# pigimonaco/Pinocchio

Measured on AMD Instinct MI355X. Metric: grid-cells/sec for full Fmax sweep (all smoothing radii) + 3LPT, 1024^3 box, higher is better.
Workload: dtype f64

## Files before the change

include/pinfmax.h:

```cpp
#ifndef PINFMAX_H
#define PINFMAX_H

#include <stddef.h>
#include <stdint.h>

#ifdef __cplusplus
extern "C" {
#endif

#define PF_NBINS 210
#define PF_MAX_SMOOTH 64

typedef struct pf_ctx pf_ctx;

typedef struct {
  int64_t n;
  int     rank;
  int     nranks;
  int     device;
  int     field_bytes;
  int     flags;
} pf_config;

#define PF_FLAG_TIMING 1
// ... 212 lines not shown
int pf_debug_pk(int which, const float *a, const float *b, float *out, int count);
int pf_debug_gfft(int n, int dir, const double *in, double *out);
int pf_debug_gfft_lines(int n, int mode, int dir, int nlines, const double *in, double *out);
int pf_debug_strided_jobs(int field_bytes, int n, int njobs, int nin, const int *in_of, const int *mul, int nouter, int ncols,
                          const double *in, double *out);
int pf_debug_strided_band(int field_bytes, int n, int njobs, int nin, const int *in_of, const int *mul, int nouter, int ncols,
                          int in_pitch, int out_pitch, int band_e, int band_outer, int outer_offset, int pre, double rs, double growth,
                          const double *in, double *out, int *guard_ok);
int pf_debug_zpass_jobs(int field_bytes, int n, int form, int njobs, const int *mul, const int *out_f32, int in_place, int nrows, int band,
                        double norm, const double *dc, int ncu, const double *spec, const double *hess, const double *acc, double *out,
                        int *sentinel_ok);
int pf_debug_strided_xfuse(int field_bytes, int n, int njobs, const int *mul, int nouter, int ncols, int pre, double rs, double growth,
                           int outer_offset, const double *in, double *out_fused, double *out_plain);
int pf_debug_invariant_reruns(pf_ctx *ctx);
int pf_solve_ran_beside_zpass(pf_ctx *ctx);
int pf_transform_path(pf_ctx *ctx);
int pf_invgrow_table_status(pf_ctx *ctx, int ismooth, double *max_rel_err);
int pf_collapse_cells(pf_ctx *ctx, int ismooth, const double *d, size_t count, double *F);
enum { PF_ARITH_FAST = 0, PF_ARITH_EXACT = 1 };
int pf_set_arithmetic(pf_ctx *ctx, int flavour);
int pf_get_arithmetic(pf_ctx *ctx);
#define PF_CENSUS_BINS 64
typedef struct {
  unsigned long long cells;
  unsigned long long differing_bits;
  unsigned long long hist[PF_CENSUS_BINS];
  unsigned long long beyond_2ulp;
  unsigned long long rmax_differing;
  unsigned long long nonfinite;
  unsigned long long outliers;
// ... 95 lines not shown
```

pinocchio_amd/_lib.py:

```python
from __future__ import annotations

import ctypes as C
import os

PKG = os.path.dirname(os.path.abspath(__file__))
SO = os.environ.get("PINFMAX_LIB") or os.path.join(PKG, "libpinfmax_hip.so")
NBINS = 210
MAX_SMOOTH = 64

FLAG_TIMING = 1
FLAG_DOUBLE_PRODUCTS = 2
MAP_CURRENT = 0
MAP_UPDATE = 1
NEIGH_SKIP, NEIGH_GOOD, NEIGH_PEAK = 1, 2, 4


class Config(C.Structure):
    _fields_ = [("n", C.c_int64), ("rank", C.c_int), ("nranks", C.c_int), ("device", C.c_int),
                ("field_bytes", C.c_int), ("flags", C.c_int)]


class ProductLayout(C.Structure):
    _fields_ = [("stride", C.c_size_t), ("off_Rmax", C.c_int), ("off_Fmax", C.c_int), ("off_Vel", C.c_int),
                ("off_Vel_2LPT", C.c_int), ("off_Vel_3LPT_1", C.c_int), ("off_Vel_3LPT_2", C.c_int)]
# ... 246 lines not shown
    "pf_debug_math": (C.c_int, [_vp, C.c_int, C.POINTER(C.c_double), C.POINTER(C.c_double), C.c_size_t, C.POINTER(C.c_double)]),
    "pf_debug_stream_rate": (C.c_int, [_vp, C.c_int, C.c_int, _dp]),
    "pf_debug_lines": (C.c_int, [C.c_int, C.c_int, C.c_int, C.c_int, C.c_int, C.c_int, C.c_int, C.c_int, C.c_double, C.c_double, C.c_int, _dp, _dp]),
    "pf_debug_pk": (C.c_int, [C.c_int, C.POINTER(C.c_float), C.POINTER(C.c_float), C.POINTER(C.c_float), C.c_int]),
    "pf_debug_gfft": (C.c_int, [C.c_int, C.c_int, _dp, _dp]),
    "pf_debug_gfft_lines": (C.c_int, [C.c_int, C.c_int, C.c_int, C.c_int, _dp, _dp]),
    "pf_debug_strided_jobs": (C.c_int, [C.c_int, C.c_int, C.c_int, C.c_int, C.POINTER(C.c_int), C.POINTER(C.c_int), C.c_int, C.c_int, _dp, _dp]),
    "pf_debug_strided_band": (C.c_int, [C.c_int, C.c_int, C.c_int, C.c_int, C.POINTER(C.c_int), C.POINTER(C.c_int), C.c_int, C.c_int, C.c_int, C.c_int,
                                        C.c_int, C.c_int, C.c_int, C.c_int, C.c_double, C.c_double, _dp, _dp, C.POINTER(C.c_int)]),
    "pf_debug_zpass_jobs": (C.c_int, [C.c_int, C.c_int, C.c_int, C.c_int, C.POINTER(C.c_int), C.POINTER(C.c_int), C.c_int, C.c_int, C.c_int, C.c_double,
                                      _dp, C.c_int, _dp, _dp, _dp, _dp, C.POINTER(C.c_int)]),
    "pf_debug_strided_xfuse": (C.c_int, [C.c_int, C.c_int, C.c_int, C.POINTER(C.c_int), C.c_int, C.c_int, C.c_int, C.c_double, C.c_double, C.c_int,
                                         _dp, _dp, _dp]),
    "pf_debug_invariant_reruns": (C.c_int, [_vp]),
    "pf_solve_ran_beside_zpass": (C.c_int, [_vp]),
    "pf_transform_path": (C.c_int, [_vp]),
    "pf_invgrow_table_status": (C.c_int, [_vp, C.c_int, _dp]),
    "pf_set_loopback_exchange": (C.c_int, [_vp, C.c_int]),
    "pf_loopback_active": (C.c_int, [_vp]),
    "pf_set_sources_in_sweep": (C.c_int, [_vp, C.c_int]),
    "pf_set_lpt_order": (C.c_int, [_vp, C.c_int]),
    "pf_set_ct_interpolation": (C.c_int, [_vp, C.c_int]),
    "pf_set_transposed_spectra": (C.c_int, [_vp, C.c_int]),
    "pf_replicated_spectrum": (C.c_int, [_vp]),
    "pf_update_products": (C.c_int, [_vp, _vp, C.POINTER(ProductLayout)]),
    "pf_set_growth_table": (C.c_int, [_vp, C.c_int, C.POINTER(C.c_double), C.c_int, C.c_double, C.c_double, C.c_double]),
    "pf_get_second_derivative": (C.c_int, [_vp, C.c_int, _dp]),
    "pf_get_kvector": (C.c_int, [_vp, C.c_int, _dp]),
    "pf_get_density": (C.c_int, [_vp, _dp]),
    "pf_debug_replicated_rows": (C.c_int, [_vp, C.c_int, C.c_int, _dp]),
# ... 73 lines not shown
```

pinocchio_amd/csrc/pf_api.hip:

```cpp
#include <hip/hip_runtime.h>

#include <math.h>
#include <stdarg.h>
#include <stdio.h>
#include <stdlib.h>
#include <string.h>

#include <atomic>
#include <string>
#include <functional>
#include <vector>

#include "../../include/pinfmax.h"
#include "pf_collapse_core.h"
#include "pf_hostpool.h"
#include "pf_internal.h"

extern "C" void pf_rccl_release(void *link);
extern "C" int pf_rccl_link_count(void *link);

static thread_local char g_err[512] = "";
int pf_fail(int task, const char *fmt, ...) {
  va_list ap;
  va_start(ap, fmt);
// ... 110 lines not shown
  int tab_ns;
  double tab_var[PF_MAX_SMOOTH];
  bool tab_ready;
  int tab_ismooth;
  int tab_built_fast;
  int model;
  double sng_cosmo[7], sng_Din[PF_MAX_SMOOTH], sng_size[PF_MAX_SMOOTH];
  int sng_ns;
  PfCtDev ct;
  double *ct_block;
  bool have_density, have_hessian, have_sources, products_init;
  int sources_order;
  bool sweep_sources, sources_fresh;
  bool x_pending[3];
  bool s3b_start_absent;
  bool transposed;
  int ct_flavour;
  int lpt_order;
  void *plc = nullptr;
  double *partials_src;
  bool general;
  void *W;
  void *fft_c2r, *fft_r2c;
  bool vel_zero_pending;
  int last_ns;
  struct PfHandoff *handoff;
  PfLoopback *loopback;
  pf_alltoall_fn a2a; void *a2a_user;
  pf_alltoallv_fn a2av; void *a2av_user;
  pf_allreduce_fn ared; void *ared_user;
// ... 110 lines not shown
  t->spline_lut = env_int("PF_SPLINE_LUT", 1) != 0;
  t->exchange_rows = env_int("PF_EXCHANGE_ROWS", 1) != 0;
  t->invariants = env_int("PF_INVARIANTS", 1);
  t->lpt_fuse = env_int("PF_LPT_FUSE", 1);
  t->collapse_wg_per_cu = env_int("PF_COLLAPSE_WG_PER_CU", 8);
  if (t->collapse_wg_per_cu <= 0) t->collapse_wg_per_cu = 8;
  t->general = env_int("PF_GENERAL", 0) != 0;

  t->pipeline = env_int("PF_PIPELINE", 1) != 0;
  t->replicate = env_int("PF_REPLICATE_DK", -1);
  t->exact_libm = env_int("PF_EXACT_LIBM", 0) != 0;
  t->solve_beside_z = env_int("PF_SOLVE_BESIDE_Z", -1);
  t->gtab = env_int("PF_GTAB", 1) != 0;
  t->lpt_xfuse = env_int("PF_LPT_XFUSE", 1) != 0;
  t->lpt3b_start = env_int("PF_LPT3B_START", 0) != 0;
  t->preflight = env_int("PF_PREFLIGHT", 1) != 0;
  t->handoff_chunk_mb = env_int("PF_HANDOFF_CHUNK_MB", 256);
  if (t->handoff_chunk_mb <= 0) t->handoff_chunk_mb = 256;
  t->handoff_threads = env_int("PF_HANDOFF_THREADS", 0);
  t->host_register = env_int("PF_HOST_REGISTER", 0) != 0;
  t->distribute_lds = env_int("PF_DISTRIBUTE_LDS", 1) != 0;
  const char *fault = getenv("PF_DEBUG_PIPELINE_FAULT");
  t->debug_fault = !fault ? 0 : !strcmp(fault, "recv") ? 1 : !strcmp(fault, "send") ? 2 : 0;
  t->prune_eps = 8.673617379884035e-19;
  if (const char *e = getenv("PF_PRUNE_EPS")) t->prune_eps = atof(e);
}

static void plan_bytes(const pf_ctx *c, size_t *at_create, size_t *peak) {
  const size_t field = c->field_bytes, nc = ncell_of(c);
  size_t fields = 1 + 3 + 6 + 3;
// ... 132 lines not shown
    return pf_fail(rank, "pf_create: PF_FLAG_DOUBLE_PRODUCTS (fp64 Fmax and displacements) needs fp64 fields");
  int ndev = 0;
  if (hipGetDeviceCount(&ndev) != hipSuccess || ndev <= 0)
    return pf_fail(rank, "pf_create: no HIP device available (libpinfmax_hip has no CPU path)");
  if (cfg->device < 0 || cfg->device >= ndev) return pf_fail(rank, "pf_create: device %d out of range (%d devices)", cfg->device, ndev);
  pf_ctx *c = new pf_ctx();
  c->cfg = *cfg; c->rank = rank; c->P = cfg->nranks; c->n = (int)n; c->nzh = c->n / 2 + 1; c->nzp = c->n / 2 + 64 / cfg->field_bytes;
  c->tune = tune; c->dev = cfg->device; c->inv_reruns = 0;
  c->general = want_general; c->fft_c2r = c->fft_r2c = nullptr; c->W = nullptr;
  if (c->general) c->nzp = c->nzh;
  c->nxl = c->n / c->P; c->nyl = c->n / c->P; c->fb = cfg->field_bytes; c->timing = (cfg->flags & PF_FLAG_TIMING) != 0; c->pb = (cfg->flags & PF_FLAG_DOUBLE_PRODUCTS) ? 8 : 4;
  c->dev_bytes = 0; c->own_stream = true; c->stream = nullptr;
  c->a2a = nullptr; c->a2av = nullptr; c->a2av_user = nullptr; c->ared = nullptr; c->a2a_user = c->ared_user = nullptr; c->rccl = nullptr;
  c->have_density = c->have_hessian = c->have_sources = c->products_init = false; c->last_ns = 0;
  c->sweep_sources = c->sources_fresh = false; c->x_pending[0] = c->x_pending[1] = c->x_pending[2] = false; c->s3b_start_absent = false; c->partials_src = nullptr; c->lpt_order = 3; c->ct_flavour = 0; c->transposed = false;
  c->vel_zero_pending = false; c->have_genic = false;
  memset(c->ks_ms, 0, sizeof(c->ks_ms)); memset(c->ks_bytes, 0, sizeof(c->ks_bytes)); memset(c->ks_n, 0, sizeof(c->ks_n));
  memset(&c->cpu, 0, sizeof(c->cpu)); memset(c->spl_set, 0, sizeof(c->spl_set)); memset(c->spl_n, 0, sizeof(c->spl_n));
  c->growth[0] = 1.0; c->growth[1] = 3. / 7.; c->growth[2] = -1. / 9.; c->growth[3] = 5. / 42.;
  for (int i = 0; i < 6; i++) { c->B[i] = nullptr; c->B2[i] = nullptr; }
  c->blockA = nullptr; c->dk = nullptr; c->recvA = nullptr; c->tw = nullptr;
  c->blockA2 = nullptr; c->recvA2 = nullptr; c->cstream = nullptr; c->dk_full = nullptr; c->replicate = false; c->dk_full_valid = false; for (int k = 0; k < 3; k++) c->INV[0][k] = c->INV[1][k] = nullptr; c->inv_w = 0; c->inv_own[0] = c->inv_own[1] = nullptr; c->blockS = c->blockB2 = nullptr;
  c->fmax = nullptr; c->rmax = nullptr; c->vel12 = nullptr; c->back_zacc = nullptr; c->back_group = nullptr; c->vel12_prev = nullptr; c->prev_shifts = 0; c->have_displacements = false; c->partials = nullptr; c->scal = nullptr; c->hist = nullptr; c->spl = nullptr;
  c->gtab = nullptr; c->etab = nullptr; c->ct_block = nullptr; c->gt = nullptr; c->gt_lut = nullptr;
  memset(c->gt_ok, 0, sizeof(c->gt_ok)); memset(c->gt_err, 0, sizeof(c->gt_err));
  for (int i = 0; i < 2; i++) c->ev_x[i] = c->ev_r[i] = c->ev_y[i] = c->ev_s[i] = nullptr;
  c->sstream = nullptr; c->solve_ran_beside = false; c->loopback = nullptr; c->handoff = nullptr;
  c->pipeline = c->P > 1 && tune.pipeline;
  for (int i = 0; i < 3; i++) { c->A[i] = nullptr; c->S[i] = nullptr; }
  memset(c->gt_n, 0, sizeof(c->gt_n));
  c->tab_ns = 0; c->tab_ready = false; c->tab_ismooth = -1; c->tab_built_fast = -1; c->model = 0; c->sng_ns = 0; memset(c->sng_cosmo, 0, sizeof(c->sng_cosmo)); memset(c->sng_size, 0, sizeof(c->sng_size)); memset(&c->ct, 0, sizeof(c->ct));
// ... 327 lines not shown
    }
    KTimer t(c, KS_ZPASS_INV, njobs * frac_in * spec_bytes_alg(c) + 3.0 * (double)ncell(c) * 8.0);
    PFCHK(c, pf_launch_c2r_invariants(c->fb, c->n, p, c->stream));
    return 0;
  }
  KTimer t(c, kind, njobs * frac_in * spec_bytes_alg(c) + outb);
  PFCHK(c, pf_launch_c2r(c->fb, c->n, p, c->stream));
  return 0;
}

__global__ void k_debug_idle(long long ticks) {
  const long long t0 = wall_clock64();
  while (wall_clock64() - t0 < ticks) __builtin_amdgcn_s_sleep(32);
}
template <class Pre, class Dst, class Post, class Band>
static int pipelined_band(pf_ctx *c, int count, int nf, Pre pre, Dst dst, Post post, Band band, bool local = false) {
  void *A[2][3];
  const void *R[3];
  if (local) {
    for (int i = 0; i < count; i++) {
      void *D[3];
      for (int f = 0; f < nf; f++) { D[f] = dst(i, 0, f); R[f] = D[f]; }
      if (pre(i, D)) return 1;
      if (post(i, R)) return 1;
    }
    return 0;
  }
  for (int f = 0; f < 3; f++) { A[0][f] = c->A[f]; A[1][f] = c->pipeline ? (void *)(c->blockA2 + f * c->field_bytes) : c->A[f]; }
  if (c->P == 1 || !c->pipeline) {
    for (int i = 0; i < count; i++) {
      if (pre(i, A[0])) return 1;
      for (int f = 0; f < nf; f++) {
        R[f] = A[0][f];
        if (c->P > 1) { void *d = dst(i, 0, f); PFCHK(c, exchange_band(c, A[0][f], d, band(i))); R[f] = d; }
      }
      if (post(i, R)) return 1;
    }
    return 0;
  }
  auto issue = [&](int i) -> int {
    const int s = i & 1;
    if (c->tune.debug_fault == 2) hipLaunchKernelGGL(k_debug_idle, dim3(1), dim3(1), 0, c->stream, 200000LL);
    if (pre(i, A[s])) return 1;
    HIPCHK(c, hipEventRecord(c->ev_x[s], c->stream));
    if (c->tune.debug_fault != 2) HIPCHK(c, hipStreamWaitEvent(c->cstream, c->ev_x[s], 0));
// ... 80 lines not shown
    const double kb = kc * c->n / (2.0 * 3.14159265358979323846);
    if (kb < c->n / 2 - 1) band = (int)kb + 1;
  }
  return band;
}
static int x_pending_of(const pf_ctx *c, const void *spec) {
  for (int i = 0; i < 3; i++) if (c->x_pending[i] && spec == c->S[i]) return i;
  return -1;
}
static int finish_forward_x(pf_ctx *c, int i) {
  const Job xj[1] = {{c->S[i], c->S[i], PF_MUL_ONE}};
  PFCHK(c, xpass(c, KS_XPASS_FWD, -1, 1, xj, 0, 0.0, 1.0, 1));
  c->x_pending[i] = false;
  return 0;
}
static int hess_x(pf_ctx *c, const void *spec, double rs, void *const A[3], int band, bool replicated = false) {
  const Job xj[3] = {{spec, A[0], PF_MUL_ONE}, {spec, A[1], PF_MUL_K}, {spec, A[2], PF_MUL_K2}};
  int pend = replicated ? -1 : x_pending_of(c, spec);
  if (pend >= 0 && band < c->n / 2) { PFCHK(c, finish_forward_x(c, pend)); pend = -1; }
  return xpass(c, KS_XPASS_HESS, +1, 3, xj, 1, rs, 1.0, 1, band, true, replicated, pend >= 0);
}
static int ensure_dk_full(pf_ctx *c) {
  if (!c->replicate || c->dk_full_valid) return 0;
  if (c->a2a == loopback_a2a && c->have_genic) {
    unsigned int *dseed = nullptr;
    const int rc = pf_genic_launch(c->fb, c->dk_full, c->n, c->nzp, c->n, 0, &c->genic, c->stream, &dseed);
    if (!rc) HIPCHK(c, hipStreamSynchronize(c->stream));
    hipFree(dseed);
    if (rc) return pf_fail(c->rank, "pf_genic_density (whole spectrum): launch failed");
    c->dk_full_valid = true;
    return 0;
  }
  const size_t rows = (size_t)c->nyl * c->nzp * 2 * c->fb;
  HIPCHK(c, hipMemsetAsync(c->dk_full, 0, (size_t)c->P * c->field_bytes, c->stream));
  HIPCHK(c, hipMemcpy2DAsync((char *)c->dk_full + (size_t)c->rank * rows, (size_t)c->P * rows, c->dk, rows, rows, (size_t)c->n,
                             hipMemcpyDeviceToDevice, c->stream));
  PFCHK(c, allreduce_dev(c, c->dk_full, (size_t)c->P * c->field_bytes / 8, 1));
  c->dk_full_valid = true;
  return 0;
}
static int hess_yz(pf_ctx *c, const void *const R[3], const double *dc, void *const out[6], int band, bool invariants = false,
                   void *acc = nullptr, void *const *hfirst = nullptr, bool in_local = false, const std::function<int()> *between = nullptr) {
  const Job yj[6] = {{R[2], out[0], PF_MUL_ONE}, {R[1], out[3], PF_MUL_K}, {R[1], out[4], PF_MUL_ONE},
                     {R[0], out[1], PF_MUL_K2}, {R[0], out[5], PF_MUL_K},  {R[0], out[2], PF_MUL_ONE}};
  PFCHK(c, ypass(c, KS_YPASS_HESS, +1, 6, yj, true, false, 3, band, true, in_local));
  if (between && (*between)()) return 1;
  const ZJob zj[6] = {{out[0], out[0], PF_MUL_ONE, 0}, {out[1], out[1], PF_MUL_ONE, 0}, {out[2], out[2], PF_MUL_K2, 0},
                      {out[3], out[3], PF_MUL_ONE, 0}, {out[4], out[4], PF_MUL_K, 0},   {out[5], out[5], PF_MUL_K, 0}};
  if (acc) {
    ZJob cj[6];
    for (int i = 0; i < 6; i++) { cj[i] = zj[i]; cj[i].out = hfirst[i]; }
    PFCHK(c, zpass_c2r(c, KS_ZPASS_HESS, 6, cj, dc, band, false, acc));
    return 0;
  }
  PFCHK(c, zpass_c2r(c, KS_ZPASS_HESS, 6, zj, dc, band, invariants));
  return 0;
}
static int hessian_of(pf_ctx *c, const void *spec, double rs, const double *dc, void *const out[6],
                      void *acc = nullptr, void *const *hfirst = nullptr) {
  if (c->general) return g_hessian_of(c, spec, rs, out);
// ... 149 lines not shown
static int dc_of_host_spec(pf_ctx *c, const double *host, int slot) {
  const double dcv = (c->rank == 0) ? host[0] / ((double)c->n * c->n * c->n) : 0.0;
  HIPCHK(c, hipMemcpyAsync(c->scal + slot, &dcv, sizeof(double), hipMemcpyHostToDevice, c->stream));
  HIPCHK(c, hipStreamSynchronize(c->stream));
  PFCHK(c, allreduce_dev(c, c->scal + slot, 1, 0));
  HIPCHK(c, hipStreamSynchronize(c->stream));
  return 0;
}

extern "C" int pf_set_density(pf_ctx *c, const double *kd) {
  if (!c || !kd) return pf_fail(0, "pf_set_density: null argument");
  PhaseTimer pt(c, 3);
  PFCHK(c, import_spec(c, kd, c->dk));
  PFCHK(c, dc_of_host_spec(c, kd, SC_DC_DK));
  c->have_genic = false;
  c->have_density = true; c->have_hessian = false; c->have_sources = false; c->sources_fresh = false; c->dk_full_valid = false;
  return 0;
}

extern "C" int pf_synth_density(pf_ctx *c, uint64_t seed, double sigma0, double slope) {
  if (!c) return 1;
  if (c->general) {
    PFCHK(c, pf_launch_white(c->fb, c->B[0], (long long)c->n * c->n, 0, c->n, c->n, seed, c->stream));
    PFCHK(c, g_r2c(c, c->B[0], c->dk));
  } else {
    PFCHK(c, pf_launch_white(c->fb, c->dk, (long long)c->nxl * c->n, (long long)c->rank * c->nxl * c->n, c->n, 2 * c->nzp, seed, c->stream));
    PFCHK(c, forward_of(c, c->dk));
  }
  PfShapeParams p; memset(&p, 0, sizeof(p));
  p.spec = c->dk; p.n = c->n; p.nzp = c->nzp; p.nyl = c->nyl; p.y0 = c->rank * c->nyl; p.slope = slope; p.scale = 1.0;
  p.partials = c->partials; p.nblocks = PF_NBLK; p.mode = 0; p.dscale = nullptr;
  PFCHK(c, pf_launch_shape(c->fb, p, c->stream));
  PFCHK(c, pf_launch_sum1(c->partials, PF_NBLK, 1.0, c->scal + SC_POWER, c->stream));
  PFCHK(c, allreduce_dev(c, c->scal + SC_POWER, 1, 0));
  PFCHK(c, pf_launch_sigma_scale(c->scal + SC_POWER, sigma0, (double)c->n * c->n * c->n, c->scal + SC_DSCALE, c->stream));
  p.mode = 1; p.dscale = c->scal + SC_DSCALE;
  PFCHK(c, pf_launch_shape(c->fb, p, c->stream));
  HIPCHK(c, hipMemsetAsync(c->scal + SC_DC_DK, 0, sizeof(double), c->stream));
  HIPCHK(c, hipStreamSynchronize(c->stream));
  c->have_genic = false;
  c->have_density = true; c->have_hessian = false; c->have_sources = false; c->sources_fresh = false; c->dk_full_valid = false;
  return 0;
}

extern "C" int pf_genic_density(pf_ctx *c, const pf_genic_params *p) {
  if (!c || !p) return pf_fail(0, "pf_genic_density: null argument");
  if (!(p->BoxSize_true_Mpc > 0) || !(p->PkNorm > 0) || !(p->Omega0 > 0) || !(p->Hubble100 > 0))
    return pf_fail(c->rank, "pf_genic_density: BoxSize, PkNorm, Omega0 and Hubble100 must be positive");
  unsigned int *dseed = nullptr;
  if (pf_genic_launch(c->fb, c->dk, c->n, c->nzp, c->nyl, c->rank * c->nyl, p, c->stream, &dseed)) {
    hipFree(dseed);
    return pf_fail(c->rank, "pf_genic_density: launch failed");
  }
  HIPCHK(c, hipMemsetAsync(c->scal + SC_DC_DK, 0, sizeof(double), c->stream));
  HIPCHK(c, hipStreamSynchronize(c->stream));
  hipFree(dseed);
  c->genic = *p;
  if (p->pk_n > 0 && p->pk_logk && p->pk_logk3p) {
    c->genic_logk.assign(p->pk_logk, p->pk_logk + p->pk_n); c->genic_logk3p.assign(p->pk_logk3p, p->pk_logk3p + p->pk_n);
    c->genic.pk_logk = c->genic_logk.data(); c->genic.pk_logk3p = c->genic_logk3p.data();
  }
  c->have_genic = true;
  c->have_density = true; c->have_hessian = false; c->have_sources = false; c->sources_fresh = false; c->dk_full_valid = false;
  return 0;
}

extern "C" int pf_set_invgrow(pf_ctx *c, int ismooth, const double *x, const double *y, int n) {
  if (!c || !x || !y) return pf_fail(0, "pf_set_invgrow: null argument");
  if (n < 3 || n > PF_KNOT_CAP) return pf_fail(c->rank, "pf_set_invgrow: %d knots not in [3, %d]", n, PF_KNOT_CAP);
  if (ismooth < -1 || ismooth >= PF_MAX_SMOOTH) return pf_fail(c->rank, "pf_set_invgrow: ismooth %d out of range", ismooth);
  for (int i = 1; i < n; i++)
    if (!(x[i] > x[i - 1])) return pf_fail(c->rank, "pf_set_invgrow: knots must be strictly increasing (i=%d)", i);
  std::vector<double> h(5 * PF_KNOT_CAP, 0.0);
  memcpy(&h[0], x, n * sizeof(double));
  memcpy(&h[PF_KNOT_CAP], y, n * sizeof(double));
  if (pf_spline_coeffs(x, y, n, &h[2 * PF_KNOT_CAP])) return pf_fail(c->rank, "pf_set_invgrow: spline set-up failed");
  pf_spline_bd(x, y, &h[2 * PF_KNOT_CAP], n, &h[3 * PF_KNOT_CAP], &h[4 * PF_KNOT_CAP]);
  const int slot = ismooth + 1;
// ... 21 lines not shown
static int spline_for(pf_ctx *c, int ismooth, PfSplineDev *s) {
  int slot = (ismooth >= 0 && ismooth < PF_MAX_SMOOTH && c->spl_set[ismooth + 1]) ? ismooth + 1 : 0;
  if (!c->spl_set[slot]) return pf_fail(c->rank, "inverse-growth spline not set (pf_set_invgrow)");
  const double *t = c->spl + (size_t)slot * 5 * PF_KNOT_CAP;
  s->x = t; s->y = t + PF_KNOT_CAP; s->c = t + 2 * PF_KNOT_CAP; s->b = t + 3 * PF_KNOT_CAP; s->d = t + 4 * PF_KNOT_CAP;
  s->n = c->spl_n[slot];
  const bool gt = c->gt_ok[slot] && c->tune.gtab;
  s->gt = gt ? c->gt + (size_t)slot * PF_GT_DOUBLES : nullptr;
  s->gt_lut = gt ? c->gt_lut + (size_t)slot * PF_GT_MAX_BINS : nullptr;
  return 0;
}

extern "C" int pf_set_growth(pf_ctx *c, const double g[4]) {
  if (!c || !g) return 1;
  memcpy(c->growth, g, 4 * sizeof(double));
  return 0;
}

extern "C" int pf_set_growth_table(pf_ctx *c, int order, const double *log10_growth, int nk, double logkmin, double dlogk, double sign) {
  if (!c || order < 1 || order > 4) return pf_fail(0, "pf_set_growth_table: order must be 1..4");
  if (nk < 0 || nk == 1 || nk > PF_KBIN_CAP || (nk && !log10_growth)) return pf_fail(c->rank, "pf_set_growth_table: %d k-bins not in {0, 2..%d}", nk, PF_KBIN_CAP);
  const int o = order - 1;
  if (nk) HIPCHK(c, hipMemcpyAsync(c->gtab + o * PF_KBIN_CAP, log10_growth, nk * sizeof(double), hipMemcpyHostToDevice, c->stream));
  HIPCHK(c, hipStreamSynchronize(c->stream));
  c->gt_n[o] = nk; c->gt_logkmin[o] = logkmin; c->gt_dlogk[o] = dlogk; c->gt_sign[o] = sign;
  return 0;
}

static int ct_alloc(pf_ctx *c) {
  if (c->ct_block) return 0;
  const size_t nd = PF_CT_NBINS_D, nt = (size_t)PF_CT_NBINS_D * PF_CT_NBINS_XY * PF_CT_NBINS_XY;
  PFCHK(c, dev_alloc(c, (void **)&c->ct_block, (3 * nd + 4 * nt) * sizeof(double)));
  double h[3 * PF_CT_NBINS_D];
  memset(h, 0, sizeof(h));
  pf_ct_delta_vector(h);
  pf_ct_tridiag(h, PF_CT_NBINS_D, h + nd, h + 2 * nd);
  HIPCHK(c, hipMemcpy(c->ct_block, h, sizeof(h), hipMemcpyHostToDevice));
  c->ct.delta = c->ct_block; c->ct.alpha = c->ct_block + nd; c->ct.gamma = c->ct_block + 2 * nd;
  c->ct.y = c->ct_block + 3 * nd; c->ct.b = c->ct.y + nt; c->ct.c = c->ct.b + nt; c->ct.d = c->ct.c + nt;
  return 0;
// ... 124 lines not shown
             (double)ncell(c) * ((invariants ? 3.0 * 8.0 / c->fb : sources ? (p.src[2] ? 9.0 : 8.0) : 6.0) * c->fb + 16.0), st);
    PFCHK(c, pf_launch_collapse(solve_fb, p, st));
  }
  PFCHK(c, pf_launch_final_sum(c->partials, p.nblocks, c->scal + SC_VAR0 + 2 * ismooth, st));
  if (sources) {
    PFCHK(c, pf_launch_sum1(c->partials_src, p.nblocks, 1.0 / ((double)c->n * c->n * c->n), c->scal + SC_DC_S2, st));
    c->sources_fresh = true;
  }
  return 0;
}

static int products_reset(pf_ctx *c) {
  c->vel_zero_pending = true;
  c->products_init = true;
  c->have_displacements = false;
  return 0;
}
static int velocities_ready(pf_ctx *c) {
  if (c->vel_zero_pending) {
    HIPCHK(c, hipMemsetAsync(c->vel12, 0, 12 * ncell(c) * (size_t)c->pb, c->stream));
    c->vel_zero_pending = false;
  }
  return 0;
}

extern "C" int pf_collapse_times(pf_ctx *c, int ismooth, double *tv) {
  if (!c) return 1;
  if (!c->have_hessian) return pf_fail(c->rank, "pf_collapse_times: second derivatives not computed");
  if (ismooth < 0 || ismooth >= PF_MAX_SMOOTH) return pf_fail(c->rank, "pf_collapse_times: ismooth %d out of range", ismooth);
  if (ismooth == 0) {
    PFCHK(c, products_reset(c));
  } else if (!c->products_init)
    return pf_fail(c->rank, "pf_collapse_times: products not initialised (ismooth 0 must come first)");
  {
    PhaseTimer pt(c, 1);
    if (collapse_enqueue(c, ismooth, c->B, c->stream, !(c->tab_ready && c->tab_ismooth == ismooth))) return 1;
// ... 25 lines not shown
  const bool invariants_ok = (c->tune.invariants >= 2 ? pf_c2r_invariants_supported(c->fb, (int)c->n) : pf_c2r_invariants_preferred(c->fb, (int)c->n)) && !c->general && c->tab_ns == 0 && c->model == 0 && c->tune.invariants && !six_components;
  HIPCHK(c, hipMemsetAsync(c->scal + SC_INV_FLAG, 0, sizeof(double), c->stream));
  const bool rep = c->replicate;
  if (rep) PFCHK(c, ensure_dk_full(c));
  bool beside_z = invariants_ok && (c->tune.solve_beside_z < 0 ? c->fb == 4 : c->tune.solve_beside_z != 0);
  if (beside_z && c->fb == 8 && ensure_b2(c, true)) beside_z = false;
  if (beside_z && c->fb == 4 && inv_rows(c, 1, true)) beside_z = false;
  const bool two_field_sets = beside_z && c->fb == 8;
  struct { bool valid; int ismooth, set; } pending = {false, 0, 0};
  bool s_live[2] = {false, false};
  auto join_solves = [&]() -> int {
    for (int k = 0; k < 2; k++)
      if (s_live[k]) { HIPCHK(c, hipStreamWaitEvent(c->stream, c->ev_s[k], 0)); s_live[k] = false; }
    return 0;
  };
  auto pre = [&](int ismooth, void *const *A) {
    PhaseTimer pt(c, 0);
    return hess_x(c, rep ? c->dk_full : c->dk, radius_cells[ismooth], A, hess_band(c, radius_cells[ismooth]), rep);
  };
  auto post = [&](int ismooth, const void *const *R) {
    const bool inv = invariants_ok && ismooth < ns - 1;
    const bool side = inv && beside_z;
    const int set = side ? (ismooth & 1) : 0;
    void *const *H = set && two_field_sets ? c->B2 : c->B;
    auto fields_of = [&](int s_) -> void *const * { return s_ && two_field_sets ? c->B2 : c->B; };
    if (pending.valid && !side) {
      if (join_solves()) return 1;
      PhaseTimer pt(c, 1);
      if (collapse_enqueue(c, pending.ismooth, fields_of(pending.set), c->stream, true, true, false, pending.set)) return 1;
      pending.valid = false;
    }
    if (s_live[set]) {
      HIPCHK(c, hipStreamWaitEvent(c->stream, c->ev_s[set], 0));
// ... 2 lines not shown
    const std::function<int()> between = [&]() -> int {
      if (!pending.valid) return 0;
      const int ps = pending.set;
      HIPCHK(c, hipEventRecord(c->ev_y[ps], c->stream));
      HIPCHK(c, hipStreamWaitEvent(c->sstream, c->ev_y[ps], 0));
      {
        PhaseTimer pt(c, 1, c->sstream);
        if (collapse_enqueue(c, pending.ismooth, fields_of(ps), c->sstream, true, true, false, ps)) return 1;
      }
      HIPCHK(c, hipEventRecord(c->ev_s[ps], c->sstream));
      s_live[ps] = true;
      pending.valid = false;
      return 0;
    };
    c->inv_w = set;
    {
      PhaseTimer pt(c, 0);
      PFCHK(c, hess_yz(c, R, c->scal + SC_DC_DK, H, hess_band(c, radius_cells[ismooth]), inv, nullptr, nullptr, rep, side ? &between : nullptr));
    }
    c->inv_w = 0;
    if (side) {
      pending.valid = true; pending.ismooth = ismooth; pending.set = set;
      return 0;
    }
    if (join_solves()) return 1;
    PhaseTimer pt(c, 1);
    return collapse_enqueue(c, ismooth, c->B, c->stream, true, inv, c->sweep_sources && ismooth == ns - 1);
  };
  if (c->general) {
    for (int ismooth = 0; ismooth < ns; ismooth++) {
      {
        PhaseTimer pt(c, 0);
        PFCHK(c, g_hessian_of(c, c->dk, radius_cells[ismooth], c->B));
      }
      PhaseTimer pt(c, 1);
      if (collapse_enqueue(c, ismooth, c->B, c->stream, true, false, c->sweep_sources && ismooth == ns - 1)) return 1;
    }
  } else if (pipelined_band(c, ns, 3, pre, [&](int, int set, int f) { return recv_field(c, set, f); }, post,
                            [&](int ismooth) { return hess_band(c, radius_cells[ismooth]); }, rep)) return 1;
  c->solve_ran_beside = beside_z && ns > 2;
  if (pending.valid) return pf_fail(c->rank, "pf_sweep: a solve was left waiting (internal error)");
  if (join_solves()) return 1;
  c->have_hessian = true; c->last_ns = ns;
  PFCHK(c, allreduce_dev(c, c->scal + SC_INV_FLAG, 1 + 2 * (size_t)ns, 0));
  std::vector<double> s(1 + 2 * ns);
  HIPCHK(c, hipMemcpyAsync(s.data(), c->scal + SC_INV_FLAG, s.size() * sizeof(double), hipMemcpyDeviceToHost, c->stream));
  HIPCHK(c, hipStreamSynchronize(c->stream));
  if (true_variance)
    for (int i = 0; i < ns; i++) true_variance[i] = s[1 + 2 * i + 1] / ((double)c->n * c->n * c->n);
  return s[0] != 0.0 ? 2 : 0;
}

extern "C" int pf_sweep(pf_ctx *c, int ns, const double *radius_cells, double *true_variance) {
  if (!c || !radius_cells) return pf_fail(0, "pf_sweep: null argument");
// ... 33 lines not shown
  arithmetic_set(c, !own_fast);
  int rc = pf_sweep(c, ns, radius_cells, true_variance);
  arithmetic_set(c, own_fast);
  if (rc) return rc;
  HIPCHK(c, hipMemcpyAsync(sh.f, c->fmax, nc * (size_t)c->pb, hipMemcpyDeviceToDevice, c->stream));
  HIPCHK(c, hipMemcpyAsync(sh.r, c->rmax, nc * sizeof(int), hipMemcpyDeviceToDevice, c->stream));
  rc = pf_sweep(c, ns, radius_cells, true_variance);
  if (rc) return rc;
  const void *ff = own_fast ? c->fmax : sh.f, *fe = own_fast ? sh.f : c->fmax;
  const int *rf = own_fast ? c->rmax : sh.r, *re = own_fast ? sh.r : c->rmax;
  KTimer t(c, KS_MISC, (double)nc * (2.0 * c->pb + 8.0));
  return pf_census_device(who, c->rank, c->pb, 0, nc, ff, rf, fe, re, out, capacity, cells, c->stream);
}
extern "C" int pf_debug_invariant_reruns(pf_ctx *c) { return c ? c->inv_reruns : -1; }
extern "C" int pf_solve_ran_beside_zpass(pf_ctx *c) { return c ? (c->solve_ran_beside ? 1 : 0) : -1; }
extern "C" int pf_replicated_spectrum(pf_ctx *c) { return c ? (c->replicate ? 1 : 0) : -1; }
extern "C" int pf_transform_path(pf_ctx *c) { return !c ? -1 : c->general ? 2 : (c->n & (c->n - 1)) ? 1 : 0; }
extern "C" int pf_set_transposed_spectra(pf_ctx *c, int on) {
  if (!c) return 1;
  c->transposed = on != 0;
  return 0;
}
extern "C" int pf_set_ct_interpolation(pf_ctx *c, int flavour) {
  if (!c) return 1;
  if (flavour < 0 || flavour > 2) return pf_fail(c->rank, "pf_set_ct_interpolation: flavour %d (0 BILINEAR_SPLINE, 1 TRILINEAR, 2 ALL_SPLINE)", flavour);
  c->ct_flavour = flavour;
  return 0;
}
extern "C" int pf_set_lpt_order(pf_ctx *c, int order) {
  if (!c) return 1;
  if (order < 1 || order > 3) return pf_fail(c->rank, "pf_set_lpt_order: order %d (1 Zel'dovich, 2 -DTWO_LPT, 3 -DTHREE_LPT)", order);
  c->lpt_order = order;
  return 0;
}
extern "C" int pf_set_sources_in_sweep(pf_ctx *c, int on) {
  if (!c) return 1;
  c->sweep_sources = on != 0;
  return 0;
}

extern "C" int pf_displacements(pf_ctx *c, int compute_sources, int recompute_sd) {
  if (!c) return 1;
  if (!c->have_density) return pf_fail(c->rank, "pf_displacements: density not set");
  if (ensure_b2(c)) return 1;
  if (!c->products_init) {
    PFCHK(c, pf_launch_fill_products(c->fmax, c->rmax, c->vel12, ncell(c), c->pb, c->stream));
    c->products_init = true;
  }
  if (recompute_sd && c->lpt_order >= 2) {
    PhaseTimer pt(c, 0);
    PFCHK(c, hessian_of(c, c->dk, 0.0, c->scal + SC_DC_DK, c->B));
    c->have_hessian = true; c->sources_fresh = false;
  }
  {
    PhaseTimer pt(c, 2);
    if (compute_sources && c->lpt_order >= 2) {
      if (!c->have_hessian) return pf_fail(c->rank, "pf_displacements: second derivatives at R=0 not in place");
      if (!c->sources_fresh) {
      c->s3b_start_absent = false;
// ... 24 lines not shown
        for (int i = 0; i < 6; i++) { ap.h[i] = c->B[i]; ap.phi2[i] = c->B2[i]; }
        ap.s3b = c->S[2]; ap.pitch = rpitch(c); ap.nrows = (long long)c->nxl * c->n; ap.n = c->n;
        KTimer t(c, KS_LPT_ACC, 14.0 * real_bytes_alg(c));
        PFCHK(c, pf_launch_lpt_accum(c->fb, ap, c->stream));
      }
      void *const s12[2] = {c->S[1], c->S[2]};
      if (c->lpt_order >= 3) PFCHK(c, forward_many(c, 2, s12));
      c->have_sources = true; c->sources_order = c->lpt_order;
    } else if (c->lpt_order >= 2 && (!c->have_sources || c->sources_order < c->lpt_order))
      return pf_fail(c->rank, "pf_displacements: LPT sources not resident (call with compute_sources = 1 first)");
    void *tmp[3] = {c->B2[0], c->B2[1], c->B2[2]};
    const void *specs[4];
    int orders[4], count = 0;
    if (c->lpt_order >= 2) { specs[count] = c->S[0]; orders[count++] = 1; }
    if (c->lpt_order >= 3) { specs[count] = c->S[1]; orders[count++] = 2; specs[count] = c->S[2]; orders[count++] = 3; }
    specs[count] = c->dk; orders[count++] = 0;
    PFCHK(c, displacements_of(c, count, specs, orders, tmp));
    if (c->lpt_order < 3) {
      const size_t nc = ncell(c);
      const int k0 = c->lpt_order == 2 ? 6 : 3;
      HIPCHK(c, hipMemsetAsync(velcol(c, k0), 0, (size_t)(12 - k0) * nc * (size_t)c->pb, c->stream));
    }
    c->vel_zero_pending = false;
    c->have_displacements = true;
  }
  return 0;
}

extern "C" int pf_fmax_pdf(pf_ctx *c, unsigned long long hist[PF_NBINS]) {
  if (!c || !hist) return 1;
  HIPCHK(c, hipMemsetAsync(c->hist, 0, PF_NBINS * sizeof(unsigned long long), c->stream));
  PFCHK(c, pf_launch_fmax_pdf(c->fmax, ncell(c), c->hist, c->pb, c->stream));
// ... 1255 lines not shown
```

pinocchio_amd/csrc/pf_internal.h:

```cpp
#pragma once
#include <hip/hip_runtime.h>
#include <stddef.h>
#include <stdint.h>

#include "../../include/pinfmax.h"

#define PF_MAX_JOBS 6
#define PF_MAX_DEVICES 64

struct PfTuning {
  int zpass_persist;
  int zpass_inv_wg_per_cu;
  int collapse_wg_per_cu;
  bool spline_lut, exchange_rows, general, pipeline, exact_libm;
  int invariants, lpt_fuse;
  int replicate;
  double prune_eps;
  int debug_fault;
  int solve_beside_z;
  int handoff_chunk_mb, handoff_threads;
  bool host_register;
  bool preflight;
  bool distribute_lds;
  bool gtab;
  bool lpt3b_start;
  bool lpt_xfuse;
};

enum { PF_MUL_ONE = 0, PF_MUL_K = 1, PF_MUL_K2 = 2, PF_MUL_IK = 3 };

struct PfAddr {
  long long os;
  int el_shift;
  long long ehs, els;
  int el_len;
};

struct PfStridedJob {
  const void *in;
  void *out;
  int mul;
// ... 297 lines not shown
```

Measured before the change: 1.528 billion.

## Share Zel'dovich displacement transforms with the final unsmoothed Hessian sweep pass

When the last smoothing radius is zero, the x-pass of the Hessian also produces an i·k-multiplied field, and the y/z passes then produce the first-order displacement columns directly. pf_displacements later skips the separate inverse transform of the density for the Zel'dovich term. The aim is to save one full 3D inverse FFT set over the 1024^3 grid. In exchange it adds freshness-tracking state, borrows the S buffers as scratch, and restricts the path to single-rank or replicated runs with a unit growth factor.

New measurement: 1.523 billion. About the same (-0.3%).

```diff
diff --git a/include/pinfmax.h b/include/pinfmax.h
--- a/include/pinfmax.h
+++ b/include/pinfmax.h
@@ -250,6 +250,7 @@
                            int outer_offset, const double *in, double *out_fused, double *out_plain);
 int pf_debug_invariant_reruns(pf_ctx *ctx);
 int pf_solve_ran_beside_zpass(pf_ctx *ctx);
+int pf_debug_zel_shared(pf_ctx *ctx);
 int pf_transform_path(pf_ctx *ctx);
 int pf_invgrow_table_status(pf_ctx *ctx, int ismooth, double *max_rel_err);
 int pf_collapse_cells(pf_ctx *ctx, int ismooth, const double *d, size_t count, double *F);
diff --git a/pinocchio_amd/_lib.py b/pinocchio_amd/_lib.py
--- a/pinocchio_amd/_lib.py
+++ b/pinocchio_amd/_lib.py
@@ -284,6 +284,7 @@
                                          _dp, _dp, _dp]),
     "pf_debug_invariant_reruns": (C.c_int, [_vp]),
     "pf_solve_ran_beside_zpass": (C.c_int, [_vp]),
+    "pf_debug_zel_shared": (C.c_int, [_vp]),
     "pf_transform_path": (C.c_int, [_vp]),
     "pf_invgrow_table_status": (C.c_int, [_vp, C.c_int, _dp]),
     "pf_set_loopback_exchange": (C.c_int, [_vp, C.c_int]),
diff --git a/pinocchio_amd/csrc/pf_api.hip b/pinocchio_amd/csrc/pf_api.hip
--- a/pinocchio_amd/csrc/pf_api.hip
+++ b/pinocchio_amd/csrc/pf_api.hip
@@ -148,6 +148,7 @@
   bool sweep_sources, sources_fresh;
   bool x_pending[3];
   bool s3b_start_absent;
+  bool zel_fresh, zel_shared;
   bool transposed;
   int ct_flavour;
   int lpt_order;
@@ -288,6 +289,7 @@
   t->gtab = env_int("PF_GTAB", 1) != 0;
   t->lpt_xfuse = env_int("PF_LPT_XFUSE", 1) != 0;
   t->lpt3b_start = env_int("PF_LPT3B_START", 0) != 0;
+  t->zel_share = env_int("PF_ZEL_SHARE", 1) != 0;
   t->preflight = env_int("PF_PREFLIGHT", 1) != 0;
   t->handoff_chunk_mb = env_int("PF_HANDOFF_CHUNK_MB", 256);
   if (t->handoff_chunk_mb <= 0) t->handoff_chunk_mb = 256;
@@ -450,7 +452,7 @@
   c->a2a = nullptr; c->a2av = nullptr; c->a2av_user = nullptr; c->ared = nullptr; c->a2a_user = c->ared_user = nullptr; c->rccl = nullptr;
   c->have_density = c->have_hessian = c->have_sources = c->products_init = false; c->last_ns = 0;
   c->sweep_sources = c->sources_fresh = false; c->x_pending[0] = c->x_pending[1] = c->x_pending[2] = false; c->s3b_start_absent = false; c->partials_src = nullptr; c->lpt_order = 3; c->ct_flavour = 0; c->transposed = false;
-  c->vel_zero_pending = false; c->have_genic = false;
+  c->vel_zero_pending = false; c->have_genic = false; c->zel_fresh = c->zel_shared = false;
   memset(c->ks_ms, 0, sizeof(c->ks_ms)); memset(c->ks_bytes, 0, sizeof(c->ks_bytes)); memset(c->ks_n, 0, sizeof(c->ks_n));
   memset(&c->cpu, 0, sizeof(c->cpu)); memset(c->spl_set, 0, sizeof(c->spl_set)); memset(c->spl_n, 0, sizeof(c->spl_n));
   c->growth[0] = 1.0; c->growth[1] = 3. / 7.; c->growth[2] = -1. / 9.; c->growth[3] = 5. / 42.;
@@ -808,21 +810,25 @@
   while (wall_clock64() - t0 < ticks) __builtin_amdgcn_s_sleep(32);
 }
 template <class Pre, class Dst, class Post, class Band>
-static int pipelined_band(pf_ctx *c, int count, int nf, Pre pre, Dst dst, Post post, Band band, bool local = false) {
-  void *A[2][3];
-  const void *R[3];
+static int pipelined_band(pf_ctx *c, int count, int nf, Pre pre, Dst dst, Post post, Band band, bool local = false, int item4 = -1, void *extra = nullptr) {
+  void *A[2][4];
+  const void *R[4];
+  if (item4 >= 0 && (nf != 3 || (c->P > 1 && !local))) return pf_fail(c->rank, "internal: a fourth field goes with three others and is never exchanged");
   if (local) {
     for (int i = 0; i < count; i++) {
-      void *D[3];
+      void *D[4];
       for (int f = 0; f < nf; f++) { D[f] = dst(i, 0, f); R[f] = D[f]; }
+      D[3] = i == item4 ? extra : nullptr; R[3] = D[3];
       if (pre(i, D)) return 1;
       if (post(i, R)) return 1;
     }
     return 0;
   }
   for (int f = 0; f < 3; f++) { A[0][f] = c->A[f]; A[1][f] = c->pipeline ? (void *)(c->blockA2 + f * c->field_bytes) : c->A[f]; }
+  A[0][3] = A[1][3] = nullptr; R[3] = nullptr;
   if (c->P == 1 || !c->pipeline) {
     for (int i = 0; i < count; i++) {
+      A[0][3] = i == item4 ? extra : nullptr; R[3] = A[0][3];
       if (pre(i, A[0])) return 1;
       for (int f = 0; f < nf; f++) {
         R[f] = A[0][f];
@@ -933,11 +939,11 @@
   c->x_pending[i] = false;
   return 0;
 }
-static int hess_x(pf_ctx *c, const void *spec, double rs, void *const A[3], int band, bool replicated = false) {
-  const Job xj[3] = {{spec, A[0], PF_MUL_ONE}, {spec, A[1], PF_MUL_K}, {spec, A[2], PF_MUL_K2}};
+static int hess_x(pf_ctx *c, const void *spec, double rs, void *const A[3], int band, bool replicated = false, void *zel_ik = nullptr) {
+  const Job xj[4] = {{spec, A[0], PF_MUL_ONE}, {spec, A[1], PF_MUL_K}, {spec, A[2], PF_MUL_K2}, {spec, zel_ik, PF_MUL_IK}};
   int pend = replicated ? -1 : x_pending_of(c, spec);
   if (pend >= 0 && band < c->n / 2) { PFCHK(c, finish_forward_x(c, pend)); pend = -1; }
-  return xpass(c, KS_XPASS_HESS, +1, 3, xj, 1, rs, 1.0, 1, band, true, replicated, pend >= 0);
+  return xpass(c, KS_XPASS_HESS, +1, zel_ik ? 4 : 3, xj, 1, rs, 1.0, 1, band, true, replicated, pend >= 0);
 }
 static int ensure_dk_full(pf_ctx *c) {
   if (!c->replicate || c->dk_full_valid) return 0;
@@ -958,11 +964,22 @@
   c->dk_full_valid = true;
   return 0;
 }
+struct ZelShare { const void *r_ik; void *t0, *t1; };
 static int hess_yz(pf_ctx *c, const void *const R[3], const double *dc, void *const out[6], int band, bool invariants = false,
-                   void *acc = nullptr, void *const *hfirst = nullptr, bool in_local = false, const std::function<int()> *between = nullptr) {
+                   void *acc = nullptr, void *const *hfirst = nullptr, bool in_local = false, const std::function<int()> *between = nullptr,
+                   const ZelShare *zel = nullptr) {
   const Job yj[6] = {{R[2], out[0], PF_MUL_ONE}, {R[1], out[3], PF_MUL_K}, {R[1], out[4], PF_MUL_ONE},
                      {R[0], out[1], PF_MUL_K2}, {R[0], out[5], PF_MUL_K},  {R[0], out[2], PF_MUL_ONE}};
-  PFCHK(c, ypass(c, KS_YPASS_HESS, +1, 6, yj, true, false, 3, band, true, in_local));
+  if (!zel) PFCHK(c, ypass(c, KS_YPASS_HESS, +1, 6, yj, true, false, 3, band, true, in_local));
+  else {
+    const Job ya[4] = {yj[0], yj[1], yj[2], {zel->r_ik, zel->t0, PF_MUL_ONE}};
+    const Job yb[4] = {yj[3], yj[4], yj[5], {R[0], zel->t1, PF_MUL_IK}};
+    PFCHK(c, ypass(c, KS_YPASS_HESS, +1, 4, ya, true, false, 3, band, true, in_local));
+    PFCHK(c, ypass(c, KS_YPASS_HESS, +1, 4, yb, true, false, 1, band, true, in_local));
+    const int compact = c->pb == 8 ? 2 : 1;
+    const ZJob dj[3] = {{zel->t0, velcol(c, 0), PF_MUL_ONE, compact}, {zel->t1, velcol(c, 1), PF_MUL_ONE, compact}, {out[2], velcol(c, 2), PF_MUL_IK, compact}};
+    PFCHK(c, zpass_c2r(c, KS_ZPASS_DISP, 3, dj, nullptr));
+  }
   if (between && (*between)()) return 1;
   const ZJob zj[6] = {{out[0], out[0], PF_MUL_ONE, 0}, {out[1], out[1], PF_MUL_ONE, 0}, {out[2], out[2], PF_MUL_K2, 0},
                       {out[3], out[3], PF_MUL_ONE, 0}, {out[4], out[4], PF_MUL_K, 0},   {out[5], out[5], PF_MUL_K, 0}};
@@ -1142,7 +1159,7 @@
   PFCHK(c, import_spec(c, kd, c->dk));
   PFCHK(c, dc_of_host_spec(c, kd, SC_DC_DK));
   c->have_genic = false;
-  c->have_density = true; c->have_hessian = false; c->have_sources = false; c->sources_fresh = false; c->dk_full_valid = false;
+  c->have_density = true; c->have_hessian = false; c->have_sources = false; c->sources_fresh = false; c->dk_full_valid = false; c->zel_fresh = false;
   return 0;
 }
 
@@ -1167,7 +1184,7 @@
   HIPCHK(c, hipMemsetAsync(c->scal + SC_DC_DK, 0, sizeof(double), c->stream));
   HIPCHK(c, hipStreamSynchronize(c->stream));
   c->have_genic = false;
-  c->have_density = true; c->have_hessian = false; c->have_sources = false; c->sources_fresh = false; c->dk_full_valid = false;
+  c->have_density = true; c->have_hessian = false; c->have_sources = false; c->sources_fresh = false; c->dk_full_valid = false; c->zel_fresh = false;
   return 0;
 }
 
@@ -1189,7 +1206,7 @@
     c->genic.pk_logk = c->genic_logk.data(); c->genic.pk_logk3p = c->genic_logk3p.data();
   }
   c->have_genic = true;
-  c->have_density = true; c->have_hessian = false; c->have_sources = false; c->sources_fresh = false; c->dk_full_valid = false;
+  c->have_density = true; c->have_hessian = false; c->have_sources = false; c->sources_fresh = false; c->dk_full_valid = false; c->zel_fresh = false;
   return 0;
 }
 
@@ -1241,6 +1258,7 @@
 extern "C" int pf_set_growth(pf_ctx *c, const double g[4]) {
   if (!c || !g) return 1;
   memcpy(c->growth, g, 4 * sizeof(double));
+  c->zel_fresh = false;
   return 0;
 }
 
@@ -1251,6 +1269,7 @@
   if (nk) HIPCHK(c, hipMemcpyAsync(c->gtab + o * PF_KBIN_CAP, log10_growth, nk * sizeof(double), hipMemcpyHostToDevice, c->stream));
   HIPCHK(c, hipStreamSynchronize(c->stream));
   c->gt_n[o] = nk; c->gt_logkmin[o] = logkmin; c->gt_dlogk[o] = dlogk; c->gt_sign[o] = sign;
+  c->zel_fresh = false;
   return 0;
 }
 
@@ -1405,12 +1424,14 @@
   c->vel_zero_pending = true;
   c->products_init = true;
   c->have_displacements = false;
+  c->zel_fresh = false;
   return 0;
 }
 static int velocities_ready(pf_ctx *c) {
   if (c->vel_zero_pending) {
     HIPCHK(c, hipMemsetAsync(c->vel12, 0, 12 * ncell(c) * (size_t)c->pb, c->stream));
     c->vel_zero_pending = false;
+    c->zel_fresh = false;
   }
   return 0;
 }
@@ -1466,9 +1487,14 @@
       if (s_live[k]) { HIPCHK(c, hipStreamWaitEvent(c->stream, c->ev_s[k], 0)); s_live[k] = false; }
     return 0;
   };
+  const bool sources_here = c->sweep_sources && c->lpt_order >= 2 && !c->tab_ns && c->model != 1;
+  const bool zel = c->tune.zel_share && c->sweep_sources && !c->general && radius_cells[ns - 1] == 0.0 && c->growth[0] == 1.0 && c->gt_n[0] == 0 &&
+                   (sources_here || !c->have_sources) && (c->P == 1 || rep);
+  c->zel_fresh = false; c->zel_shared = false;
+  if (zel) c->have_sources = false;
   auto pre = [&](int ismooth, void *const *A) {
     PhaseTimer pt(c, 0);
-    return hess_x(c, rep ? c->dk_full : c->dk, radius_cells[ismooth], A, hess_band(c, radius_cells[ismooth]), rep);
+    return hess_x(c, rep ? c->dk_full : c->dk, radius_cells[ismooth], A, hess_band(c, radius_cells[ismooth]), rep, zel && ismooth == ns - 1 ? A[3] : nullptr);
   };
   auto post = [&](int ismooth, const void *const *R) {
     const bool inv = invariants_ok && ismooth < ns - 1;
@@ -1501,9 +1527,12 @@
       return 0;
     };
     c->inv_w = set;
+    const bool zel_here = zel && ismooth == ns - 1;
+    const ZelShare zs = {zel_here ? R[3] : nullptr, c->S[0], c->S[1]};
+    if (zel_here && join_solves()) return 1;
     {
       PhaseTimer pt(c, 0);
-      PFCHK(c, hess_yz(c, R, c->scal + SC_DC_DK, H, hess_band(c, radius_cells[ismooth]), inv, nullptr, nullptr, rep, side ? &between : nullptr));
+      PFCHK(c, hess_yz(c, R, c->scal + SC_DC_DK, H, hess_band(c, radius_cells[ismooth]), inv, nullptr, nullptr, rep, side ? &between : nullptr, zel_here ? &zs : nullptr));
     }
     c->inv_w = 0;
     if (side) {
@@ -1524,7 +1553,8 @@
       if (collapse_enqueue(c, ismooth, c->B, c->stream, true, false, c->sweep_sources && ismooth == ns - 1)) return 1;
     }
   } else if (pipelined_band(c, ns, 3, pre, [&](int, int set, int f) { return recv_field(c, set, f); }, post,
-                            [&](int ismooth) { return hess_band(c, radius_cells[ismooth]); }, rep)) return 1;
+                            [&](int ismooth) { return hess_band(c, radius_cells[ismooth]); }, rep, zel ? ns - 1 : -1, c->S[2])) return 1;
+  c->zel_fresh = c->zel_shared = zel;
   c->solve_ran_beside = beside_z && ns > 2;
   if (pending.valid) return pf_fail(c->rank, "pf_sweep: a solve was left waiting (internal error)");
   if (join_solves()) return 1;
@@ -1588,6 +1618,7 @@
 }
 extern "C" int pf_debug_invariant_reruns(pf_ctx *c) { return c ? c->inv_reruns : -1; }
 extern "C" int pf_solve_ran_beside_zpass(pf_ctx *c) { return c ? (c->solve_ran_beside ? 1 : 0) : -1; }
+extern "C" int pf_debug_zel_shared(pf_ctx *c) { return c ? (c->zel_shared ? 1 : 0) : -1; }
 extern "C" int pf_replicated_spectrum(pf_ctx *c) { return c ? (c->replicate ? 1 : 0) : -1; }
 extern "C" int pf_transform_path(pf_ctx *c) { return !c ? -1 : c->general ? 2 : (c->n & (c->n - 1)) ? 1 : 0; }
 extern "C" int pf_set_transposed_spectra(pf_ctx *c, int on) {
@@ -1605,6 +1636,7 @@
   if (!c) return 1;
   if (order < 1 || order > 3) return pf_fail(c->rank, "pf_set_lpt_order: order %d (1 Zel'dovich, 2 -DTWO_LPT, 3 -DTHREE_LPT)", order);
   c->lpt_order = order;
+  c->zel_fresh = false;
   return 0;
 }
 extern "C" int pf_set_sources_in_sweep(pf_ctx *c, int on) {
@@ -1617,6 +1649,8 @@
   if (!c) return 1;
   if (!c->have_density) return pf_fail(c->rank, "pf_displacements: density not set");
   if (ensure_b2(c)) return 1;
+  const bool zel_done = c->zel_fresh && compute_sources && !recompute_sd;
+  c->zel_fresh = false;
   if (!c->products_init) {
     PFCHK(c, pf_launch_fill_products(c->fmax, c->rmax, c->vel12, ncell(c), c->pb, c->stream));
     c->products_init = true;
@@ -1671,8 +1705,8 @@
     int orders[4], count = 0;
     if (c->lpt_order >= 2) { specs[count] = c->S[0]; orders[count++] = 1; }
     if (c->lpt_order >= 3) { specs[count] = c->S[1]; orders[count++] = 2; specs[count] = c->S[2]; orders[count++] = 3; }
-    specs[count] = c->dk; orders[count++] = 0;
-    PFCHK(c, displacements_of(c, count, specs, orders, tmp));
+    if (!zel_done) { specs[count] = c->dk; orders[count++] = 0; }
+    if (count) PFCHK(c, displacements_of(c, count, specs, orders, tmp));
     if (c->lpt_order < 3) {
       const size_t nc = ncell(c);
       const int k0 = c->lpt_order == 2 ? 6 : 3;
diff --git a/pinocchio_amd/csrc/pf_internal.h b/pinocchio_amd/csrc/pf_internal.h
--- a/pinocchio_amd/csrc/pf_internal.h
+++ b/pinocchio_amd/csrc/pf_internal.h
@@ -25,6 +25,7 @@
   bool gtab;
   bool lpt3b_start;
   bool lpt_xfuse;
+  bool zel_share;
 };
 
 enum { PF_MUL_ONE = 0, PF_MUL_K = 1, PF_MUL_K2 = 2, PF_MUL_IK = 3 };
```
